# Niccolo-Ajroldi/plainLM

Hardware: AMD Instinct MI355X
Metric: tokens/sec fwd+bwd (160M, seq=1024, bf16) (higher is better)
Workload: dtype bf16

## Files before the change

plainlm_amd/_lib.py:

```python

import ctypes as C
import os
import re

_HERE = os.path.dirname(os.path.abspath(__file__))
LIB_PATH = os.path.join(_HERE, 'libplainlm_hip.so')
HEADER_PATH = os.path.join(os.path.dirname(_HERE), 'include', 'plainlm_hip.h')
EXT_HEADER_PATH = os.path.join(os.path.dirname(_HERE), 'include', 'plainlm_hip_ext.h')

_lib = None

EXPECTED_ABI = 112

_P = C.c_void_p
_I64 = C.c_int64
_I = C.c_int
_F = C.c_float
_SZ = C.c_size_t

class CastItem(C.Structure):
  _fields_ = [('src', _P), ('dst', _P), ('dst_t', _P), ('rows', _I64), ('cols', _I64), ('ld_t', _I64)]


class OptimItem(C.Structure):
  _fields_ = [('p', _P), ('g', _P), ('m', _P), ('v', _P), ('dst', _P), ('dst_t', _P), ('rows', _I64), ('cols', _I64), ('ld_t', _I64)]


class OptimHparams(C.Structure):
  _fields_ = [('kind', _I), ('first', _I), ('lr', _F), ('weight_decay', _F), ('decay', _F), ('beta1', _F), ('beta2', _F), ('eps', _F),
              ('momentum', _F), ('dampening', _F), ('bc2', _F), ('coef_grad', _F), ('coef_avg', _F),
              ('ckp1', _F), ('coef_y', _F), ('bc1', _F)]
# ... 72 lines not shown
  'plm_set_cu_reserve': (_I, [_I]),
  'plm_comm_unique_id': (_I, [_P]),
  'plm_comm_init': (_I, [C.POINTER(_P), _P, _I, _I, _I]),
  'plm_comm_init_capped': (_I, [C.POINTER(_P), _P, _I, _I, _I, _I]),
  'plm_comm_split': (_I, [_P, C.POINTER(_P), _I]),
  'plm_comm_destroy': (_I, [_P]),
  'plm_comm_allreduce_avg_f32': (_I, [_P, _P, _I64, _P]),
  'plm_comm_rsag_avg_f32': (_I, [_P, _P, _I64, _P]),
  'plm_comm_broadcast_f32': (_I, [_P, _P, _I64, _I, _P]),
  'plm_mx_quant': (_I, [_P, _I64, _I64, _I64, _P, _P, _P, _P, _P]),
  'plm_mx_quant_multi': (_I, [C.POINTER(MxQuantItem), _I, _P]),
  'plm_gemm_mx_nt': (_I, [_P, _P, _P, _P, _P, _I64, _I64, _I64, _I64, _I, _P]),
  'plm_probe_ds_read_tr16': (_I, [_P, _P]),
  'plm_probe_mfma32': (_I, [_P, _P, _P, _P]),
}


EXT_SIGNATURES = {
  'plm_head_predict_workspace_bytes': (_SZ, [_I64, _I64, _I64]),
  'plm_head_predict_bf16': (_I, [_P, _I64, _P, _I64, _P, _P, _P, _P, _P, _P, _I64, _I64, _I64, _P, _SZ, _P]),
}


def _declared(path):
  with open(path) as f:
    src = re.sub(r'/\*.*?\*/', '', f.read(), flags=re.S)
  return sorted(set(re.findall(r'\b(plm_[a-z0-9_]+)\s*\(', src)))


def header_functions():
  return _declared(HEADER_PATH)


def ext_header_functions():
  return _declared(EXT_HEADER_PATH)


def load():
  global _lib
  if _lib is not None:
    return _lib
  if not os.path.exists(LIB_PATH):
    raise RuntimeError(
      f'{LIB_PATH} not found: the HIP extension is not built. Run `make -C plainlm_amd/csrc` '
      '(or __graft_entry__.build()). plainlm_amd has no CPU fallback.')
  lib = C.CDLL(LIB_PATH, mode=C.RTLD_GLOBAL)
  for name, (res, args) in SIGNATURES.items():
    fn = getattr(lib, name)
    fn.restype = res
    fn.argtypes = args
  for name, (res, args) in EXT_SIGNATURES.items():
    fn = getattr(lib, name, None)
    if fn is None:
      raise RuntimeError(f'{LIB_PATH} lacks {name} (include/plainlm_hip_ext.h): rebuild it (make -C plainlm_amd/csrc)')
    fn.restype = res
    fn.argtypes = args
  got = lib.plm_version()
  if got != EXPECTED_ABI:
    raise RuntimeError(f'{LIB_PATH} reports ABI version {got}, this package was written for {EXPECTED_ABI}: '
                       'rebuild it (make -C plainlm_amd/csrc)')
  _lib = lib
  return lib


def check(rc, what):
  if rc != 0:
    msg = load().plm_last_error_string()
    raise RuntimeError(f'{what} failed (rc={rc}): {msg.decode() if msg else "?"}')
```

plainlm_amd/csrc/gemm_api.hip:

```cpp
#include <initializer_list>

#include "../../include/plainlm_hip_ext.h"
#include "gemm_launch.h"

static int g_num_cus = 0;
static int g_cu_reserve = 0;

extern "C" int plm_set_cu_reserve(int n) {
  if (n < 0 || n > 128) {
    plm_set_error("plm_set_cu_reserve: n=%d out of range 0..128", n);
    return PLM_E_INVALID;
  }
  g_cu_reserve = n;
  return PLM_OK;
}

static bool ensure_num_cus() {
  if (g_num_cus == 0) {
    int dev = 0;
    hipDeviceProp_t prop;
    if (hipGetDevice(&dev) != hipSuccess || hipGetDeviceProperties(&prop, dev) != hipSuccess) return false;
    g_num_cus = prop.multiProcessorCount > 0 ? prop.multiProcessorCount : 256;
  }
  return true;
}
// ... 103 lines not shown
    PLM_CHECK_LAUNCH("plm_fc1_swiglu_bf16");
    return PLM_OK;
  }
  if (int rc = plm_gemm_bf16_nt_ex(X, ldx, W, ldw, U, N, M, N, K, 0, 0, nullptr, 0, stream)) return rc;
  return plm_swiglu_fwd(U, ACT, M, h, stream);
}

extern "C" int plm_fc2_dx_swiglu_bwd_bf16(const uint16_t* dY, int64_t lddy, const uint16_t* W2T, int64_t ldw, const uint16_t* U, uint16_t* DU,
                                          uint16_t* scratch, int64_t M, int64_t h, int64_t K, void* stream) {
  PLM_REQUIRE(dY && W2T && U && DU, "plm_fc2_dx_swiglu_bwd_bf16: null pointer");
  PLM_REQUIRE(M > 0 && h > 0 && K > 0 && h % 8 == 0, "plm_fc2_dx_swiglu_bwd_bf16: bad shape (h %% 8 == 0)");
  if (lddy % 8 == 0 && ldw % 8 == 0 && aligned16({dY, W2T, DU}) && (reinterpret_cast<uintptr_t>(U) & 7) == 0 &&
      launch_nt_fused(NT_EPI_GLUB, GemmOperands{dY, lddy, W2T, ldw, DU, 2 * h, M, h, K, nullptr},
                      EpiArgs{const_cast<uint16_t*>(U), 2 * h, nullptr, nullptr, 0, 0}, stream)) {
    PLM_CHECK_LAUNCH("plm_fc2_dx_swiglu_bwd_bf16");
    return PLM_OK;
  }
  if (!scratch) {
    plm_set_error("plm_fc2_dx_swiglu_bwd_bf16: this shape (or PLM_GEMM_V1) takes the two-launch path and needs the M*h bf16 d(act) scratch");
    return PLM_E_WORKSPACE;
  }
  if (int rc = plm_gemm_bf16_nt_ex(dY, lddy, W2T, ldw, scratch, h, M, h, K, 0, 0, nullptr, 0, stream)) return rc;
  return plm_swiglu_bwd(scratch, U, DU, M, h, stream);
}

extern "C" size_t plm_gemm_tn_workspace_bytes(int64_t M, int64_t N, int64_t K) {
  const int slots = persistent_slots();
  if (M <= 0 || N <= 0 || K <= 0 || slots == 0) return 0;
  return tn_plan(M, N, K, slots, plan_env()).workspace_bytes;
}

extern "C" int plm_gemm_bf16_tn(const uint16_t* A, int64_t lda, const uint16_t* B, int64_t ldb, float* C, int64_t ldc, int64_t M,
                                int64_t N, int64_t K, int accumulate, const float* alpha_dev, void* workspace,
                                size_t workspace_bytes, void* stream) {
  PLM_REQUIRE(A && B && C, "plm_gemm_bf16_tn: null pointer");
  PLM_REQUIRE(M > 0 && N > 0 && K > 0 && M < (1 << 30) && N < (1 << 30) && K < (1 << 30), "plm_gemm_bf16_tn: bad shape M=%ld N=%ld K=%ld",
              (long)M, (long)N, (long)K);
  PLM_REQUIRE(M % 8 == 0 && N % 8 == 0 && lda % 8 == 0 && ldb % 8 == 0 && ldc % 4 == 0,
              "plm_gemm_bf16_tn: M, N, lda, ldb must be multiples of 8 and ldc of 4 (M=%ld N=%ld lda=%ld ldb=%ld ldc=%ld)", (long)M, (long)N,
              (long)lda, (long)ldb, (long)ldc);
  PLM_REQUIRE(((reinterpret_cast<uintptr_t>(A) | reinterpret_cast<uintptr_t>(B) | reinterpret_cast<uintptr_t>(C)) & 15) == 0,
              "plm_gemm_bf16_tn: base pointers must be 16-byte aligned");
  const int slots = persistent_slots();
  if (slots == 0) return PLM_E_HIP;
  const TnPlan p = tn_plan(M, N, K, slots, plan_env());
  if (p.splits > 1) {
// ... 166 lines not shown
```

plainlm_amd/csrc/gemm_big.hip:

```cpp
#include <stdlib.h>

#include <type_traits>
#include <utility>

#include "gemm_launch.h"

typedef __attribute__((address_space(3))) void lds_void_t;
typedef const __attribute__((address_space(1))) void gbl_void_t;

__device__ __forceinline__ void big_dma16(const void* gsrc, void* lds_wave_base) {
  __builtin_amdgcn_global_load_lds((gbl_void_t*)gsrc, (lds_void_t*)lds_wave_base, 16, 0, 0);
}
__device__ __forceinline__ int big_swz(int row, int chunk) { return row * 128 + ((chunk ^ ((row >> 1) & 7)) << 4); }

template <int N>
__device__ __forceinline__ void wait_vm() {
#ifdef PLM_DBG_DRAIN
  asm volatile("s_waitcnt vmcnt(0)" ::: "memory");
#else
  asm volatile("s_waitcnt vmcnt(%0)" ::"n"(N) : "memory");
#endif
}
template <int N0, int N1>
__device__ __forceinline__ void wait_vm_sel(int flag) {
// ... 75 lines not shown
    for (int u = 0; u < NUNIT; ++u)
      if (slot(u) == sl) return u;
    return -1;
  }
};
static_assert(NtOvlPlan<2, 3, 2>::slot(0) == 2 && NtOvlPlan<2, 3, 2>::slot(1) == 3 && NtOvlPlan<2, 3, 2>::slot(3) == 4 && NtOvlPlan<2, 3, 2>::slot(2) == 5,
              "256x192: (A0,B0) (A0,B1) (A1,B1) leave in phases 2 3 4, (A1,B0) behind the loop");
static_assert(NtOvlPlan<4, 2, 1>::slot(0) == 3 && NtOvlPlan<4, 2, 1>::slot(1) == 4 && NtOvlPlan<4, 2, 1>::slot(2) == 5 && NtOvlPlan<4, 2, 1>::slot(3) == 5,
              "256x256: the two pieces of A half 0 leave in phases 3 and 4");
static_assert(NtOvlPlan<1, 3, 2>::slot(1) == 4 && NtOvlPlan<1, 3, 2>::slot(0) == 5, "128x192: the B1 pass leaves in phase 4");

__device__ __forceinline__ float4 head_rec_combine(const float4 a, const float4 b) {
  const float m = fmaxf(a.x, b.x);
  const float ea_ = __expf(a.x - m), eb_ = __expf(b.x - m);
  const float sa = (a.x == -INFINITY) ? 0.f : a.y * ea_;
  const float sb = (b.x == -INFINITY) ? 0.f : b.y * eb_;
  const float ua = (a.x == -INFINITY) ? 0.f : ea_ * fmaf(a.y, a.x - m, a.z);
  const float ub = (b.x == -INFINITY) ? 0.f : eb_ * fmaf(b.y, b.x - m, b.z);
  const int ia = __float_as_int(a.w), ib = __float_as_int(b.w);
  const int idx = b.x > a.x ? ib : (b.x == a.x ? min(ia, ib) : ia);
  return make_float4(m, sa + sb, ua + ub, __int_as_float(idx));
}

template <int BM, int BN, int WM, int WN, bool HYB = false, bool GLU = false, bool GLUB = false, bool ROPE = false, bool SCORE = false>
__global__ __launch_bounds__(512, 2) void gemm_nt_big_kernel(const uint16_t* __restrict__ A, int64_t lda,
                                                             const uint16_t* __restrict__ B, int64_t ldb,
                                                             uint16_t* __restrict__ C, int64_t ldc, int M, int N, int K,
                                                             const float* __restrict__ alpha_dev, int tiles_m, int tiles_n,
                                                             HybridArgs hyb, EpiArgs ea) {
  uint16_t* const act = ea.act;
  const int64_t ldact = ea.ldact;
  static_assert(!(GLU || GLUB) || (BM == 256 && BN == 256 && WN == 4 && !HYB), "GLU epilogues: 256x256 tiles, whole-K items");
  static_assert(!(GLU && GLUB), "one epilogue at a time");
  static_assert(!SCORE || !(HYB || GLU || GLUB || ROPE), "SCORE: whole-K items, no other epilogue");
  constexpr int TM = BM / WM, TN = BN / WN;
  static_assert(WM * WN == 8 && (TN == 64 || TN == 96) && (TM == 128 || TM == 64 || TM == 32), "unsupported geometry");
  constexpr int AH = TM / 2;
  constexpr int NA = AH / 16;
  constexpr int BF0 = TN / 32 - 1, NBF = BF0 + 1;
  constexpr int A_ROWS = BM / 2, B0_ROWS = WN * 32 * BF0, B1_ROWS = WN * 32;
  constexpr int A_HT = A_ROWS * 128, B0_HT = B0_ROWS * 128, B1_HT = B1_ROWS * 128;
  constexpr int STAGE = 2 * A_HT + B0_HT + B1_HT;
  constexpr int A_DMA = A_ROWS / 64, B0_DMA = B0_ROWS / 64, B1_DMA = B1_ROWS / 64;
  static_assert(B0_DMA >= B1_DMA && B1_DMA >= 1, "half-tiles are whole DMA rounds of the workgroup");
  constexpr int OFF_A0 = 0, OFF_B0 = A_HT, OFF_B1 = A_HT + B0_HT, OFF_A1 = A_HT + B0_HT + B1_HT;
  constexpr int D_P4 = 2 * A_DMA + B0_DMA + 2 * B1_DMA;
  constexpr int D_P1 = 3 * A_DMA + B0_DMA + B1_DMA;
  constexpr int D_P2 = 3 * A_DMA + B0_DMA + B1_DMA;
  constexpr int NS = NA * 2 * NBF * (GLUB ? 2 : 1) + (GLU ? NA * 2 : 0);
  static_assert(D_P1 + NS < 64, "vmcnt is a 6-bit counter");
#ifndef PLM_NT_OVL
#define PLM_NT_OVL 1
#endif
  constexpr bool OVL = PLM_NT_OVL && !HYB && !GLU && !GLUB && !ROPE && !SCORE;
  using OP = NtOvlPlan<NA, NBF, BF0>;
  constexpr int NPASS = OP::NPASS, NUNIT = OP::NUNIT;
// ... 457 lines not shown
      auto drain = [&](auto utag) {
        constexpr int u = decltype(utag)::value;
        if (ovl && OP::slot(u) != 5) return;
        unit_write(utag);
        asm volatile("s_waitcnt lgkmcnt(0)" ::: "memory");
        unit_store(utag, std::false_type{}, m0, n0);
        asm volatile("s_waitcnt lgkmcnt(0)" ::: "memory");
      };
      nt_for_units(drain, std::make_integer_sequence<int, NUNIT>{});
      credit = m0 + BM <= M && n0 + BN <= N;
      credit_i = __builtin_amdgcn_readfirstlane(credit ? (ovl ? 2 : 1) : 0);
      continue;
    }
#pragma unroll
    for (int mf = 0; mf < NA; ++mf) {
      const int mrow0 = m0 + wm * TM + mf * 32;
      if (GLUB) {
        const uint16_t* u = act;
#pragma unroll
        for (int sr = 0; sr < 2; ++sr) {
          const int gm_l = min(mrow0 + sr * 16 + l15, M - 1);
          const int fi = 2 * mf + sr;
#pragma unroll
          for (int bq = 0; bq < 2; ++bq)
#pragma unroll
            for (int sc = 0; sc < 2; ++sc) {
              const int gn = n0 + wn * TN + bq * 32 + sc * 16 + 4 * q;
              const bf16x4_t xv = ld_bf16x4(u + (int64_t)gm_l * ldact + gn);
              const bf16x4_t zv = ld_bf16x4(u + (int64_t)gm_l * ldact + N + gn);
              bf16x4_t dxo, dzo;
#pragma unroll
              for (int e = 0; e < 4; ++e) {
                const float gf = bf2f(f2bf(acc4[fi][bq * 2 + sc][e]));
                const float xf = bf2f(xv[e]), zf = bf2f(zv[e]);
                const float sig = plm_sigmoid(xf);
                const bf16_t sv = f2bf(xf * sig);
                const bf16_t ds = f2bf(gf * zf);
                dzo[e] = f2bf(gf * bf2f(sv));
                dxo[e] = f2bf(bf2f(ds) * (sig * (1.f + xf * (1.f - sig))));
              }
              const int c = bq * 4 + sc * 2 + (q >> 1);
              *reinterpret_cast<bf16x4_t*>(epi + l15 * 128 + ((c ^ (l15 & 7)) << 4) + (q & 1) * 8) = dxo;
              *reinterpret_cast<bf16x4_t*>(epi + (16 + l15) * 128 + ((c ^ (l15 & 7)) << 4) + (q & 1) * 8) = dzo;
            }
          asm volatile("s_waitcnt lgkmcnt(0)" ::: "memory");
#pragma unroll
          for (int it = 0; it < 4; ++it) {
            const int c = it * 64 + lane;
            const int row = c >> 3, ch = c & 7;
            const bf16x8_t v = *reinterpret_cast<const bf16x8_t*>(epi + row * 128 + ((ch ^ (row & 7)) << 4));
            const int gm = mrow0 + sr * 16 + (row & 15);
            if (gm < M) st_c2_bf16x8(C + (int64_t)gm * ldc + (row >> 4) * N + n0 + wn * TN + ch * 8, v);
          }
          asm volatile("s_waitcnt lgkmcnt(0)" ::: "memory");
        }
        continue;
      }
#pragma unroll
      for (int p0 = 0; p0 < NBF; p0 += 2) {
        const int nb = NBF - p0 < 2 ? NBF - p0 : 2;
#pragma unroll
        for (int bq = 0; bq < 2; ++bq) {
          if (bq >= nb) continue;
          const int bh = p0 + bq;
#pragma unroll
          for (int sr = 0; sr < 2; ++sr)
#pragma unroll
            for (int sc = 0; sc < 2; ++sc) {
              bf16x4_t o;
#pragma unroll
              for (int e = 0; e < 4; ++e) o[e] = f2bf(acc4[2 * mf + sr][bh * 2 + sc][e]);
              const int row = sr * 16 + l15, c = bq * 4 + sc * 2 + (q >> 1);
              *reinterpret_cast<bf16x4_t*>(epi + row * 128 + ((c ^ (row & 7)) << 4) + (q & 1) * 8) = o;
            }
        }
        asm volatile("s_waitcnt lgkmcnt(0)" ::: "memory");
#pragma unroll
        for (int it = 0; it < 4; ++it) {
          if (it >= 2 * nb) continue;
          const int c = it * 64 + lane;
          const int row = nb == 2 ? c >> 3 : c >> 2, ch = nb == 2 ? c & 7 : c & 3;
          const bf16x8_t v = *reinterpret_cast<const bf16x8_t*>(epi + row * 128 + ((ch ^ (row & 7)) << 4));
// ... 424 lines not shown
  const int nq = N >> 3;
  const int64_t nv = (int64_t)rows * nq;
  const int64_t stride = (int64_t)gridDim.x * blockDim.x;
  for (int64_t i = (int64_t)blockIdx.x * blockDim.x + threadIdx.x; i < nv; i += stride) {
    const int64_t row = i / nq;
    const int col = (int)(i - row * nq) * 8;
    const int t = (int)(row >> 8) * tiles_n + (col >> 8);
    const int cf = (t * nkt) / L;
    const int cl = min(((t + 1) * nkt - 1) / L, nchunks - 1);
    f32x4_t a = *reinterpret_cast<const f32x4_t*>(ws + row * N + col);
    f32x4_t b = *reinterpret_cast<const f32x4_t*>(ws + row * N + col + 4);
    for (int k = 1; k <= cl - cf; ++k) {
      a += *reinterpret_cast<const f32x4_t*>(ws + ((int64_t)k * rows + row) * N + col);
      b += *reinterpret_cast<const f32x4_t*>(ws + ((int64_t)k * rows + row) * N + col + 4);
    }
    u32x4_t o = {pack_bf2(a[0] * alpha, a[1] * alpha), pack_bf2(a[2] * alpha, a[3] * alpha), pack_bf2(b[0] * alpha, b[1] * alpha),
                 pack_bf2(b[2] * alpha, b[3] * alpha)};
    *reinterpret_cast<u32x4_t*>(C + row * ldc + col) = o;
  }
}

template <NtEpilogue EPI, bool HYB, int BM, int BN, int WM, int WN>
static void nt_launch_tile(const NtPlan& p, const GemmOperands& o, float* slabs, const EpiArgs& ea, hipStream_t s) {
  hipLaunchKernelGGL((gemm_nt_big_kernel<BM, BN, WM, WN, HYB, EPI == NT_EPI_GLU, EPI == NT_EPI_GLUB, EPI == NT_EPI_ROPE, EPI == NT_EPI_SCORE>),
                     dim3((unsigned)p.grid), dim3(512), 0, s, o.A, o.lda, o.B, o.ldb, (uint16_t*)o.C, o.ldc, (int)o.M, (int)o.N, (int)o.K, o.alpha_dev, p.tm,
                     p.tn, HybridArgs{p.rfull, p.nchunks, p.L, slabs}, ea);
}

template <NtEpilogue EPI>
static void nt_launch(const NtPlan& p, const GemmOperands& o, float* slabs, const EpiArgs& ea, hipStream_t s) {
  if constexpr (EPI == NT_EPI_NONE) {
    if (p.kernel == NT_HYBRID) {
      nt_launch_tile<EPI, true, 256, 256, 2, 4>(p, o, slabs, ea, s);
      const int64_t rem_rows = o.M - (int64_t)p.rfull * 256;
      const int64_t nv = rem_rows * (o.N / 8);
      int64_t rb = plm_cdiv(nv, 256);
      if (rb > 4096) rb = 4096;
      hipLaunchKernelGGL(nt_streamk_reduce_kernel, dim3((unsigned)rb), dim3(256), 0, s, (const float*)slabs,
                         (uint16_t*)o.C + (int64_t)p.rfull * 256 * o.ldc, o.ldc, (int)rem_rows, (int)o.N, p.tn, (int)(o.K / 64), p.L, p.nchunks, o.alpha_dev);
      return;
    }
  }
  if (p.tile == 0) nt_launch_tile<EPI, false, 256, 256, 2, 4>(p, o, nullptr, ea, s);
  if constexpr (EPI != NT_EPI_GLU && EPI != NT_EPI_GLUB) {
    if (p.tile == 1) nt_launch_tile<EPI, false, 256, 128, 4, 2>(p, o, nullptr, ea, s);
    else if (p.tile == 2) nt_launch_tile<EPI, false, 256, 192, 4, 2>(p, o, nullptr, ea, s);
    else if (p.tile == 3) nt_launch_tile<EPI, false, 128, 192, 4, 2>(p, o, nullptr, ea, s);
  }
}

void plm_launch_gemm_nt_persistent(const NtPlan& p, NtEpilogue epilogue, const GemmOperands& o, float* slabs, const EpiArgs& ea, hipStream_t s) {
  switch (epilogue) {
    case NT_EPI_NONE: return nt_launch<NT_EPI_NONE>(p, o, slabs, ea, s);
    case NT_EPI_ROPE: return nt_launch<NT_EPI_ROPE>(p, o, slabs, ea, s);
    case NT_EPI_GLU: return nt_launch<NT_EPI_GLU>(p, o, slabs, ea, s);
    case NT_EPI_GLUB: return nt_launch<NT_EPI_GLUB>(p, o, slabs, ea, s);
    case NT_EPI_SCORE: return nt_launch<NT_EPI_SCORE>(p, o, slabs, ea, s);
  }
}

__global__ __launch_bounds__(256) void head_score_combine_kernel(const float* __restrict__ part, const float* __restrict__ xt,
                                                                 const int64_t* __restrict__ targets, float* __restrict__ nll,
                                                                 float* __restrict__ lse_out, int M, int V, int ntc) {
  __shared__ float2 sh[8][32];
  const int r = threadIdx.x & 31, sl = threadIdx.x >> 5;
  const int row = blockIdx.x * 32 + r;
  float m = -INFINITY, s = 0.f;
  if (row < M) {
    for (int tc = sl; tc < ntc; tc += 8) {
      const float2 b = *reinterpret_cast<const float2*>(part + 2 * ((int64_t)tc * M + row));
      const float mm = fmaxf(m, b.x);
      const float sa = (m == -INFINITY) ? 0.f : s * __expf(m - mm);
      const float sb = (b.x == -INFINITY) ? 0.f : b.y * __expf(b.x - mm);
      m = mm;
      s = sa + sb;
    }
  }
  sh[sl][r] = make_float2(m, s);
  __syncthreads();
  if (sl != 0 || row >= M) return;
#pragma unroll
// ... 117 lines not shown
```

plainlm_amd/csrc/gemm_launch.h:

```cpp
#pragma once

#include "gemm_plan.h"
#include "plm_device.h"

struct EpiArgs {
  uint16_t* act;
  int64_t ldact;
  const float* rcos;
  const float* rsin;
  int T, rope_cols;
  const int64_t* targets;
  float* part;
  float* xt;
  float* part4;
};

struct GemmOperands {
  const uint16_t* A;
  int64_t lda;
  const uint16_t* B;
  int64_t ldb;
  void* C;
  int64_t ldc, M, N, K;
  const float* alpha_dev;
};

void plm_launch_gemm_nt_128(const NtPlan& p, const GemmOperands& o, int c_dtype, int accumulate, hipStream_t s);
void plm_launch_gemm_tn_128(const TnPlan& p, const GemmOperands& o, int accumulate, float* slabs, hipStream_t s);
void plm_launch_splitk_reduce(const TnPlan& p, const GemmOperands& o, int accumulate, float* slabs, hipStream_t s);

void plm_launch_gemm_nt_persistent(const NtPlan& p, NtEpilogue epilogue, const GemmOperands& o, float* slabs, const EpiArgs& ea, hipStream_t s);
void plm_launch_gemm_tn_persistent(const TnPlan& p, const GemmOperands& o, int accumulate, float* slabs, hipStream_t s);
void plm_launch_gemm_tn_grouped(const TnGroup& g, const TnGroupOut& out, int64_t K, float* ws, int slots, hipStream_t s);
void plm_launch_head_score_combine(const float* part, const float* xt, const int64_t* targets, float* nll, float* lse, int64_t M, int64_t V, int ntc,
                                   hipStream_t s);
void plm_launch_head_score_rows(const uint16_t* logits, int64_t ld, const int64_t* targets, float* nll, float* lse, int64_t rows, int64_t V,
                                hipStream_t s);
struct HeadPredictOut {
  int64_t* pred;
  float *logp, *entropy, *nll, *lse;
};
void plm_launch_head_predict_combine(const float* part4, const float* xt, const int64_t* targets, const HeadPredictOut& out, int64_t M, int64_t V,
                                     int ntc, hipStream_t s);
void plm_launch_head_predict_rows(const uint16_t* logits, int64_t ld, const int64_t* targets, const HeadPredictOut& out, int64_t rows, int64_t V,
                                  hipStream_t s);
```

plainlm_amd/csrc/gemm_plan.h:

```cpp
#pragma once

#include <stddef.h>
#include <stdint.h>

static inline int64_t plan_cdiv(int64_t a, int64_t b) { return (a + b - 1) / b; }

struct GemmPlanEnv {
  bool gemm_v1, tn_no_big, nt_no_hybrid;
  long long nt_hybrid_min_k;
};

static inline double round_efficiency(int64_t tiles, int slots) {
  const int64_t rounds = (tiles + slots - 1) / slots;
  return (double)tiles / (double)(rounds * slots);
}

struct NtTileShape {
  int bm, bn;
  double rate;
};
static const NtTileShape kNtTiles[4] = {{256, 256, 1.0}, {256, 128, 0.88}, {256, 192, 0.94}, {128, 192, 0.72}};
static const int kNtTileVariant[4] = {4, 6, 5, 7};
static inline double nt_tile_eff(int i, int64_t M, int64_t N, int slots) {
  const NtTileShape& t = kNtTiles[i];
  const int64_t tm = plan_cdiv(M, t.bm), tn = plan_cdiv(N, t.bn);
  return round_efficiency(tm * tn, slots) * ((double)N / (double)(tn * t.bn)) * ((double)M / (double)(tm * t.bm)) * t.rate;
}
static inline int nt_pick_tile(int64_t M, int64_t N, int slots, double* eff) {
  int best = 0;
  double be = -1.0;
  for (int i = 0; i < 4; ++i) {
    const double e = nt_tile_eff(i, M, N, slots);
    if (e > be) {
      be = e;
      best = i;
    }
  }
  *eff = be;
  return best;
}
static inline double nt_dma128_eff(int64_t M, int64_t N, int slots) {
  const int64_t tm = plan_cdiv(M, 128), tn = plan_cdiv(N, 128);
  return round_efficiency(tm * tn, 2 * slots) * ((double)N / (double)(tn * 128)) * ((double)M / (double)(tm * 128)) * 0.80;
}

static inline bool nt_dma_shape(int64_t N, int64_t K, int64_t ldc) { return (K % 64 == 0) && (N % 8 == 0) && (ldc % 8 == 0); }

enum NtEpilogue { NT_EPI_NONE, NT_EPI_ROPE, NT_EPI_GLU, NT_EPI_GLUB, NT_EPI_SCORE };
enum NtKernel {
  NT_REG128,
  NT_DMA128,
  NT_PERSISTENT,
  NT_HYBRID
};
struct NtPlan {
  bool ok;
  NtKernel kernel;
  int tile;
  int tm, tn, grid;
  int rfull, nchunks, L;
  size_t workspace_bytes;
};

static inline bool nt_hybrid_plan(int64_t M, int64_t N, int64_t K, int slots, const GemmPlanEnv& env, NtPlan* p) {
  if (env.nt_no_hybrid) return false;
  const bool mk = env.nt_hybrid_min_k >= 0;
  const int64_t min_k = mk ? env.nt_hybrid_min_k : 8192, min_l = mk ? 2 : 8;
  if (K % 64 != 0 || N % 8 != 0 || M < 2048 || N < 256 || K < min_k) return false;
  const int64_t R = plan_cdiv(M, 256), Cn = plan_cdiv(N, 256), tiles = R * Cn, nkt = K / 64;
  if (tiles <= slots) return false;
  if (round_efficiency(tiles, slots) >= 0.9) return false;
// ... 8 lines not shown
  if (L < min_l || L * 10 > nkt * 9) return false;
  p->rfull = (int)rf;
  p->L = (int)L;
  p->nchunks = (int)plan_cdiv(total, L);
  const int64_t nslabs = (nkt - 1) / L + 2;
  p->workspace_bytes = (size_t)nslabs * (size_t)(M - rf * 256) * (size_t)N * sizeof(float);
  return true;
}

static inline NtPlan nt_plan(int64_t M, int64_t N, int64_t K, int64_t ldc, int c_dtype, int variant, bool have_workspace, NtEpilogue epilogue,
                             int slots, const GemmPlanEnv& env) {
  NtPlan p{};
  p.ok = true;
  auto persistent = [&](int tile) {
    p.kernel = NT_PERSISTENT;
    p.tile = tile;
    p.tm = (int)plan_cdiv(M, kNtTiles[tile].bm);
    p.tn = (int)plan_cdiv(N, kNtTiles[tile].bn);
    p.grid = p.tm * p.tn < slots ? p.tm * p.tn : slots;
    p.rfull = p.tm;
    p.nchunks = 0;
    p.L = 1;
  };
  if (epilogue == NT_EPI_GLU || epilogue == NT_EPI_GLUB) {
    p.ok = !env.gemm_v1 && K % 64 == 0 && N % 256 == 0 && M >= 512;
    if (p.ok) persistent(0);
    return p;
  }
  const bool dma_ok = variant >= 2 || (variant == 0 && !env.gemm_v1 && nt_dma_shape(N, K, ldc));
  if (variant >= 3) {
    for (int i = 0; i < 4; ++i)
      if (kNtTileVariant[i] == (variant == 3 ? 4 : variant)) persistent(i);
    return p;
  }
  if (variant == 0 && dma_ok && c_dtype == 0) {
    if (have_workspace && epilogue == NT_EPI_NONE && nt_hybrid_plan(M, N, K, slots, env, &p)) {
      p.kernel = NT_HYBRID;
      p.tm = (int)plan_cdiv(M, 256);
      p.tn = (int)plan_cdiv(N, 256);
      const int nitems = p.rfull * p.tn + p.nchunks;
      p.grid = nitems < slots ? nitems : slots;
      return p;
    }
    double eff;
    const int tile = nt_pick_tile(M, N, slots, &eff);
    if (M >= 512 && N >= 128 && eff >= nt_dma128_eff(M, N, slots)) {
      persistent(tile);
      return p;
// ... 127 lines not shown
```

plainlm_amd/functional.py:

```python

import torch

from . import ops


class GradSink:

  def __init__(self):
    self.enabled = False
    self.written = set()
    self.on_ready = None
    self.on_queued = None
    self.dw_group_local, self.dw_group_ddp = 48, 12
    self.dw_queue_bytes_max = None
    self.dw_queue_bytes = 0
    self.dw_queue = []
    self.norm_queue = []

  def begin_window(self):
    self.flush_dw()
    self.written.clear()

  def defer_dw(self, dy, x, p):
    mx = isinstance(dy, ops.MxTensor) and isinstance(x, ops.MxTensor)
# ... 75 lines not shown
  def forward(ctx, x, weight, lin):
    wb, _ = lin.shadow()
    ctx.save_for_backward(x)
    ctx.lin = lin
    return ops.gemm_nt(x, wb)

  @staticmethod
  def backward(ctx, dy):
    (x,) = ctx.saved_tensors
    lin = ctx.lin
    dy = dy.contiguous()
    _, wbt = lin.shadow()
    dx = ops.gemm_nt(dy, wbt[:, :lin.out_features]) if ctx.needs_input_grad[0] else None
    dw = None
    if ctx.needs_input_grad[1]:
      sink, p = lin.sink, lin.weight
      if sink is not None and sink.active_for(p):
        sink.defer_dw(dy, x, p)
      else:
        dw = ops.gemm_tn(dy, x)
    return dx, dw, None


class SwiGLUMLPFn(torch.autograd.Function):

  @staticmethod
  def forward(ctx, x, w1, w2, fc1, fc2):
    w1b, _ = fc1.shadow()
    w2b, _ = fc2.shadow()
    u, act = ops.fc1_swiglu(x, w1b)
    ctx.save_for_backward(x, u, act)
    ctx.fc1, ctx.fc2 = fc1, fc2
    return ops.gemm_nt(act, w2b)

  @staticmethod
  def backward(ctx, dy):
    x, u, act = ctx.saved_tensors
    fc1, fc2 = ctx.fc1, ctx.fc2
    dy = dy.contiguous()
    _, w1t = fc1.shadow()
    _, w2t = fc2.shadow()
    du = ops.fc2_dx_swiglu_bwd(dy, w2t[:, :fc2.out_features], u)
    dw2 = dw1 = None
    if ctx.needs_input_grad[2]:
      sink, p = fc2.sink, fc2.weight
      if sink is not None and sink.active_for(p):
        sink.defer_dw(dy, act, p)
      else:
        dw2 = ops.gemm_tn(dy, act)
    dx = ops.gemm_nt(du, w1t[:, :fc1.out_features]) if ctx.needs_input_grad[0] else None
    if ctx.needs_input_grad[1]:
      sink, p = fc1.sink, fc1.weight
      if sink is not None and sink.active_for(p):
        sink.defer_dw(du, x, p)
      else:
        dw1 = ops.gemm_tn(du, x)
    return dx, dw1, dw2, None, None


class PlainMLPFn(torch.autograd.Function):

  @staticmethod
  def forward(ctx, x, w1, w2, fc1, fc2, kind):
    w1b, _ = fc1.shadow()
    w2b, _ = fc2.shadow()
# ... 354 lines not shown
```

plainlm_amd/ops.py:

```python

import collections
import ctypes as C
import os

import torch

from . import _lib

BF16 = torch.bfloat16
F32 = torch.float32


def _stream():
  return C.c_void_p(torch.cuda.current_stream().cuda_stream)


PROFILE = None
LAUNCH_HOOK = None


class _Timed:
  __slots__ = ('family', 'flops', 'start')

  def __init__(self, family, flops):
# ... 429 lines not shown
  return u, act


def fc2_dx_swiglu_bwd(dy, w2t, u):
  _need(dy, BF16, 'fc2_dx_swiglu_bwd.dy', 2)
  _need(w2t, BF16, 'fc2_dx_swiglu_bwd.w2t', 2)
  _need(u, BF16, 'fc2_dx_swiglu_bwd.u', 2)
  M, K = dy.shape
  h = w2t.shape[0]
  if w2t.shape[1] != K or u.shape != (M, 2 * h) or not u.is_contiguous() or dy.stride(1) != 1 or w2t.stride(1) != 1:
    raise ValueError('fc2_dx_swiglu_bwd: need dy [M, K], w2t [h, K], contiguous u [M, 2h]')
  du = torch.empty((M, 2 * h), dtype=BF16, device=dy.device)
  lib = _lib.load()
  _hook('gemm_nt_fused', 2.0 * M * h * K)
  with _Timed('gemm_nt_fused', 2.0 * M * h * K):
    rc = lib.plm_fc2_dx_swiglu_bwd_bf16(_p(dy), dy.stride(0), _p(w2t), w2t.stride(0), _p(u), _p(du), _p(None), M, h, K, _stream())
    if rc == -4:
      scratch = torch.empty((M, h), dtype=BF16, device=dy.device)
      rc = lib.plm_fc2_dx_swiglu_bwd_bf16(_p(dy), dy.stride(0), _p(w2t), w2t.stride(0), _p(u), _p(du), _p(scratch), M, h, K, _stream())
    _lib.check(rc, 'plm_fc2_dx_swiglu_bwd_bf16')
  return du


def rope_qk_(qkv, rope_cos, rope_sin, B, T, nh):
  _need(qkv, BF16, 'rope_qk.qkv', 2)
  hd = qkv.shape[1] // (3 * nh)
  _need(rope_cos, F32, 'rope_qk.rope_cos', 2)
  _need(rope_sin, F32, 'rope_qk.rope_sin', 2)
  if rope_cos.shape[0] < T or rope_cos.shape[1] != hd // 2:
    raise ValueError('rope_qk: RoPE table too short for T or wrong head_dim')
  _lib.check(_lib.load().plm_rope_qk(_p(qkv), _p(rope_cos), _p(rope_sin), B, T, nh, hd, _stream()), 'plm_rope_qk')
  return qkv


def qkv_rope(x, w_qkv, rope_cos, rope_sin, B, T, nh):
  _need(x, BF16, 'qkv_rope.x', 2)
  _need(w_qkv, BF16, 'qkv_rope.w', 2)
  M, K = x.shape
  N = w_qkv.shape[0]
  hd = N // (3 * nh)
  out = torch.empty((M, N), dtype=BF16, device=x.device)
  _hook('gemm_nt_fused', 2.0 * M * N * K)
  with _Timed('gemm_nt_fused', 2.0 * M * N * K):
    _lib.check(_lib.load().plm_qkv_rope_bf16(_p(x), x.stride(0), _p(w_qkv), w_qkv.stride(0), _p(out), N, M, K, _p(rope_cos),
                                             _p(rope_sin), B, T, nh, hd, _stream()), 'plm_qkv_rope_bf16')
  return out
# ... 316 lines not shown
```

Before: 1.065 million.

## Save fc1 SwiGLU output in a tile-packed layout matching the backward epilogue

Adds packed-layout variants of the fused fc1+SwiGLU forward GEMM and the fc2 dx+SwiGLU backward GEMM. The forward epilogue writes the pre-activation u per wave and lane in 1 KiB units, so the backward epilogue can read gate and up values with contiguous 16-byte loads instead of strided row loads. This is meant to cut uncoalesced global reads and store work in the GLU epilogues. It is on by default when the shape qualifies, pads M up to a multiple of 256 in the saved buffer, and adds an unpack kernel for consumers that need the plain layout.

```diff
diff --git a/include/plainlm_hip_packed.h b/include/plainlm_hip_packed.h
--- /dev/null
+++ b/include/plainlm_hip_packed.h
@@ -0,0 +1,22 @@
+#ifndef PLAINLM_HIP_PACKED_H
+#define PLAINLM_HIP_PACKED_H
+
+#include "plainlm_hip.h"
+
+#ifdef __cplusplus
+extern "C" {
+#endif
+
+size_t plm_swiglu_packed_bytes(int64_t M, int64_t h);
+int plm_swiglu_packed_ok(int64_t M, int64_t h, int64_t K_fc1, int64_t K_fc2);
+int plm_fc1_swiglu_packed_bf16(const uint16_t* X, int64_t ldx, const uint16_t* W, int64_t ldw, uint16_t* PACKED, uint16_t* ACT, int64_t M,
+                               int64_t h, int64_t K, int max_workgroups, void* stream);
+int plm_fc2_dx_swiglu_bwd_packed_bf16(const uint16_t* dY, int64_t lddy, const uint16_t* W2T, int64_t ldw, const uint16_t* PACKED,
+                                      uint16_t* DU, int64_t M, int64_t h, int64_t K, int max_workgroups, void* stream);
+int plm_swiglu_unpack_bf16(const uint16_t* PACKED, uint16_t* U, int64_t M, int64_t h, void* stream);
+
+#ifdef __cplusplus
+}
+#endif
+
+#endif
diff --git a/plainlm_amd/_lib.py b/plainlm_amd/_lib.py
--- a/plainlm_amd/_lib.py
+++ b/plainlm_amd/_lib.py
@@ -7,6 +7,7 @@
 LIB_PATH = os.path.join(_HERE, 'libplainlm_hip.so')
 HEADER_PATH = os.path.join(os.path.dirname(_HERE), 'include', 'plainlm_hip.h')
 EXT_HEADER_PATH = os.path.join(os.path.dirname(_HERE), 'include', 'plainlm_hip_ext.h')
+PACKED_HEADER_PATH = os.path.join(os.path.dirname(_HERE), 'include', 'plainlm_hip_packed.h')
 
 _lib = None
 
@@ -125,6 +126,15 @@
 }
 
 
+PACKED_SIGNATURES = {
+  'plm_swiglu_packed_bytes': (_SZ, [_I64, _I64]),
+  'plm_swiglu_packed_ok': (_I, [_I64, _I64, _I64, _I64]),
+  'plm_fc1_swiglu_packed_bf16': (_I, [_P, _I64, _P, _I64, _P, _P, _I64, _I64, _I64, _I, _P]),
+  'plm_fc2_dx_swiglu_bwd_packed_bf16': (_I, [_P, _I64, _P, _I64, _P, _P, _I64, _I64, _I64, _I, _P]),
+  'plm_swiglu_unpack_bf16': (_I, [_P, _P, _I64, _I64, _P]),
+}
+
+
 def _declared(path):
   with open(path) as f:
     src = re.sub(r'/\*.*?\*/', '', f.read(), flags=re.S)
@@ -137,6 +147,10 @@
 
 def ext_header_functions():
   return _declared(EXT_HEADER_PATH)
+
+
+def packed_header_functions():
+  return _declared(PACKED_HEADER_PATH)
 
 
 def load():
@@ -152,12 +166,13 @@
     fn = getattr(lib, name)
     fn.restype = res
     fn.argtypes = args
-  for name, (res, args) in EXT_SIGNATURES.items():
-    fn = getattr(lib, name, None)
-    if fn is None:
-      raise RuntimeError(f'{LIB_PATH} lacks {name} (include/plainlm_hip_ext.h): rebuild it (make -C plainlm_amd/csrc)')
-    fn.restype = res
-    fn.argtypes = args
+  for header, table in (('plainlm_hip_ext.h', EXT_SIGNATURES), ('plainlm_hip_packed.h', PACKED_SIGNATURES)):
+    for name, (res, args) in table.items():
+      fn = getattr(lib, name, None)
+      if fn is None:
+        raise RuntimeError(f'{LIB_PATH} lacks {name} (include/{header}): rebuild it (make -C plainlm_amd/csrc)')
+      fn.restype = res
+      fn.argtypes = args
   got = lib.plm_version()
   if got != EXPECTED_ABI:
     raise RuntimeError(f'{LIB_PATH} reports ABI version {got}, this package was written for {EXPECTED_ABI}: '
diff --git a/plainlm_amd/csrc/gemm_api.hip b/plainlm_amd/csrc/gemm_api.hip
--- a/plainlm_amd/csrc/gemm_api.hip
+++ b/plainlm_amd/csrc/gemm_api.hip
@@ -1,6 +1,7 @@
 #include <initializer_list>
 
 #include "../../include/plainlm_hip_ext.h"
+#include "../../include/plainlm_hip_packed.h"
 #include "gemm_launch.h"
 
 static int g_num_cus = 0;
@@ -150,6 +151,66 @@
   }
   if (int rc = plm_gemm_bf16_nt_ex(dY, lddy, W2T, ldw, scratch, h, M, h, K, 0, 0, nullptr, 0, stream)) return rc;
   return plm_swiglu_bwd(scratch, U, DU, M, h, stream);
+}
+
+static bool launch_nt_packed(NtEpilogue epilogue, const GemmOperands& o, const EpiArgs& ea, int max_workgroups, void* stream) {
+  const int slots = persistent_slots();
+  if (slots == 0) return false;
+  NtPlan p = nt_plan(o.M, o.N, o.K, o.ldc, 0, 0, false, epilogue, slots, plan_env());
+  if (!p.ok) {
+    plm_set_error("packed SwiGLU GEMM: needs K %% 64 == 0, h %% 256 == 0 and the LDS-DMA kernels (no PLM_GEMM_V1); M=%ld N=%ld K=%ld", (long)o.M, (long)o.N,
+                  (long)o.K);
+    return false;
+  }
+  if (max_workgroups > 0 && max_workgroups < p.grid) p.grid = max_workgroups;
+  plm_launch_gemm_nt_persistent(p, epilogue, o, nullptr, ea, (hipStream_t)stream);
+  return true;
+}
+
+extern "C" size_t plm_swiglu_packed_bytes(int64_t M, int64_t h) { return (M > 0 && h > 0 && h % 128 == 0) ? glu_packed_bytes(M, h) : 0; }
+
+extern "C" int plm_swiglu_packed_ok(int64_t M, int64_t h, int64_t K_fc1, int64_t K_fc2) {
+  const int slots = persistent_slots();
+  if (slots == 0 || M <= 0 || h <= 0 || K_fc1 <= 0 || K_fc2 <= 0) return 0;
+  return nt_plan(M, 2 * h, K_fc1, 2 * h, 0, 0, false, NT_EPI_GLU, slots, plan_env()).ok &&
+         nt_plan(M, h, K_fc2, 2 * h, 0, 0, false, NT_EPI_GLUB, slots, plan_env()).ok;
+}
+
+extern "C" int plm_fc1_swiglu_packed_bf16(const uint16_t* X, int64_t ldx, const uint16_t* W, int64_t ldw, uint16_t* PACKED, uint16_t* ACT, int64_t M,
+                                          int64_t h, int64_t K, int max_workgroups, void* stream) {
+  PLM_REQUIRE(X && W && PACKED && ACT, "plm_fc1_swiglu_packed_bf16: null pointer");
+  PLM_REQUIRE(M > 0 && h > 0 && K > 0 && M < (1 << 30) && h < (1 << 29) && K < (1 << 30) && h % 128 == 0,
+              "plm_fc1_swiglu_packed_bf16: bad shape (h %% 128 == 0)");
+  PLM_REQUIRE(ldx % 8 == 0 && ldw % 8 == 0 && ldx >= K && ldw >= K && aligned16({X, W, PACKED, ACT}),
+              "plm_fc1_swiglu_packed_bf16: row strides must be multiples of 8 and >= K, pointers 16-byte aligned");
+  if (!launch_nt_packed(NT_EPI_GLU_PACKED, GemmOperands{X, ldx, W, ldw, PACKED, 2 * h, M, 2 * h, K, nullptr}, EpiArgs{ACT, h, nullptr, nullptr, 0, 0},
+                        max_workgroups, stream))
+    return PLM_E_INVALID;
+  PLM_CHECK_LAUNCH("plm_fc1_swiglu_packed_bf16");
+  return PLM_OK;
+}
+
+extern "C" int plm_fc2_dx_swiglu_bwd_packed_bf16(const uint16_t* dY, int64_t lddy, const uint16_t* W2T, int64_t ldw, const uint16_t* PACKED,
+                                                 uint16_t* DU, int64_t M, int64_t h, int64_t K, int max_workgroups, void* stream) {
+  PLM_REQUIRE(dY && W2T && PACKED && DU, "plm_fc2_dx_swiglu_bwd_packed_bf16: null pointer");
+  PLM_REQUIRE(M > 0 && h > 0 && K > 0 && M < (1 << 30) && h < (1 << 29) && K < (1 << 30) && h % 256 == 0,
+              "plm_fc2_dx_swiglu_bwd_packed_bf16: bad shape (h %% 256 == 0)");
+  PLM_REQUIRE(lddy % 8 == 0 && ldw % 8 == 0 && lddy >= K && ldw >= K && aligned16({dY, W2T, PACKED, DU}),
+              "plm_fc2_dx_swiglu_bwd_packed_bf16: row strides must be multiples of 8 and >= K, pointers 16-byte aligned");
+  if (!launch_nt_packed(NT_EPI_GLUB_PACKED, GemmOperands{dY, lddy, W2T, ldw, DU, 2 * h, M, h, K, nullptr},
+                        EpiArgs{const_cast<uint16_t*>(PACKED), 2 * h, nullptr, nullptr, 0, 0}, max_workgroups, stream))
+    return PLM_E_INVALID;
+  PLM_CHECK_LAUNCH("plm_fc2_dx_swiglu_bwd_packed_bf16");
+  return PLM_OK;
+}
+
+extern "C" int plm_swiglu_unpack_bf16(const uint16_t* PACKED, uint16_t* U, int64_t M, int64_t h, void* stream) {
+  PLM_REQUIRE(PACKED && U, "plm_swiglu_unpack_bf16: null pointer");
+  PLM_REQUIRE(M > 0 && h > 0 && M < (1 << 30) && h < (1 << 29) && h % 128 == 0, "plm_swiglu_unpack_bf16: bad shape (h %% 128 == 0)");
+  PLM_REQUIRE(aligned16({PACKED}) && (reinterpret_cast<uintptr_t>(U) & 7) == 0, "plm_swiglu_unpack_bf16: PACKED must be 16-byte aligned, U 8-byte");
+  plm_launch_swiglu_unpack(PACKED, U, M, h, (hipStream_t)stream);
+  PLM_CHECK_LAUNCH("plm_swiglu_unpack_bf16");
+  return PLM_OK;
 }
 
 extern "C" size_t plm_gemm_tn_workspace_bytes(int64_t M, int64_t N, int64_t K) {
diff --git a/plainlm_amd/csrc/gemm_big.hip b/plainlm_amd/csrc/gemm_big.hip
--- a/plainlm_amd/csrc/gemm_big.hip
+++ b/plainlm_amd/csrc/gemm_big.hip
@@ -121,7 +121,7 @@
   return make_float4(m, sa + sb, ua + ub, __int_as_float(idx));
 }
 
-template <int BM, int BN, int WM, int WN, bool HYB = false, bool GLU = false, bool GLUB = false, bool ROPE = false, bool SCORE = false>
+template <int BM, int BN, int WM, int WN, bool PK = false, bool HYB = false, bool GLU = false, bool GLUB = false, bool ROPE = false, bool SCORE = false>
 __global__ __launch_bounds__(512, 2) void gemm_nt_big_kernel(const uint16_t* __restrict__ A, int64_t lda,
                                                              const uint16_t* __restrict__ B, int64_t ldb,
                                                              uint16_t* __restrict__ C, int64_t ldc, int M, int N, int K,
@@ -131,6 +131,7 @@
   const int64_t ldact = ea.ldact;
   static_assert(!(GLU || GLUB) || (BM == 256 && BN == 256 && WN == 4 && !HYB), "GLU epilogues: 256x256 tiles, whole-K items");
   static_assert(!(GLU && GLUB), "one epilogue at a time");
+  static_assert(!PK || GLU || GLUB, "PK: the packed layout of the saved fc1 output");
   static_assert(!SCORE || !(HYB || GLU || GLUB || ROPE), "SCORE: whole-K items, no other epilogue");
   constexpr int TM = BM / WM, TN = BN / WN;
   static_assert(WM * WN == 8 && (TN == 64 || TN == 96) && (TM == 128 || TM == 64 || TM == 32), "unsupported geometry");
@@ -634,17 +635,29 @@
           const int gm_l = min(mrow0 + sr * 16 + l15, M - 1);
           const int fi = 2 * mf + sr;
 #pragma unroll
-          for (int bq = 0; bq < 2; ++bq)
+          for (int bq = 0; bq < 2; ++bq) {
+            u32x4_t pg = {0u, 0u, 0u, 0u}, pu = {0u, 0u, 0u, 0u};
+            if constexpr (PK) {
+              const char* blk = reinterpret_cast<const char*>(u) +
+                                glu_packed_unit_offset(m0 / BM, 2 * (n0 / BN) + (wn >> 1), 2 * tiles_n, wm * WN + (wn & 1) * 2 + bq, mf * 4 + sr * 2);
+              pg = *reinterpret_cast<const u32x4_t*>(blk + lane * 16);
+              pu = *reinterpret_cast<const u32x4_t*>(blk + kGluPackedUnitBytes + lane * 16);
+            }
 #pragma unroll
             for (int sc = 0; sc < 2; ++sc) {
               const int gn = n0 + wn * TN + bq * 32 + sc * 16 + 4 * q;
-              const bf16x4_t xv = ld_bf16x4(u + (int64_t)gm_l * ldact + gn);
-              const bf16x4_t zv = ld_bf16x4(u + (int64_t)gm_l * ldact + N + gn);
+              bf16x4_t xv, zv;
+              if constexpr (!PK) {
+                xv = ld_bf16x4(u + (int64_t)gm_l * ldact + gn);
+                zv = ld_bf16x4(u + (int64_t)gm_l * ldact + N + gn);
+              }
               bf16x4_t dxo, dzo;
 #pragma unroll
               for (int e = 0; e < 4; ++e) {
                 const float gf = bf2f(f2bf(acc4[fi][bq * 2 + sc][e]));
-                const float xf = bf2f(xv[e]), zf = bf2f(zv[e]);
+                const unsigned wg = pg[sc * 2 + (e >> 1)], wu = pu[sc * 2 + (e >> 1)];
+                const float xf = PK ? ((e & 1) ? bf_hi(wg) : bf_lo(wg)) : bf2f(xv[e]);
+                const float zf = PK ? ((e & 1) ? bf_hi(wu) : bf_lo(wu)) : bf2f(zv[e]);
                 const float sig = plm_sigmoid(xf);
                 const bf16_t sv = f2bf(xf * sig);
                 const bf16_t ds = f2bf(gf * zf);
@@ -655,6 +668,7 @@
               *reinterpret_cast<bf16x4_t*>(epi + l15 * 128 + ((c ^ (l15 & 7)) << 4) + (q & 1) * 8) = dxo;
               *reinterpret_cast<bf16x4_t*>(epi + (16 + l15) * 128 + ((c ^ (l15 & 7)) << 4) + (q & 1) * 8) = dzo;
             }
+          }
           asm volatile("s_waitcnt lgkmcnt(0)" ::: "memory");
 #pragma unroll
           for (int it = 0; it < 4; ++it) {
@@ -668,8 +682,22 @@
         }
         continue;
       }
-#pragma unroll
-      for (int p0 = 0; p0 < NBF; p0 += 2) {
+      if constexpr (GLU && PK) {
+        char* blk = reinterpret_cast<char*>(C) + glu_packed_unit_offset(m0 / BM, n0 / BN, tiles_n, wave, mf * 4) + lane * 16;
+#pragma unroll
+        for (int sr = 0; sr < 2; ++sr)
+#pragma unroll
+          for (int g = 0; g < 2; ++g) {
+            bf16x8_t o;
+#pragma unroll
+            for (int sc = 0; sc < 2; ++sc)
+#pragma unroll
+              for (int e = 0; e < 4; ++e) o[sc * 4 + e] = f2bf(acc4[2 * mf + sr][2 * g + sc][e]);
+            st_c_bf16x8(reinterpret_cast<uint16_t*>(blk + (sr * 2 + g) * kGluPackedUnitBytes), o);
+          }
+      }
+#pragma unroll
+      for (int p0 = 0; p0 < (GLU && PK ? 0 : NBF); p0 += 2) {
         const int nb = NBF - p0 < 2 ? NBF - p0 : 2;
 #pragma unroll
         for (int bq = 0; bq < 2; ++bq) {
@@ -1140,7 +1168,9 @@
 
 template <NtEpilogue EPI, bool HYB, int BM, int BN, int WM, int WN>
 static void nt_launch_tile(const NtPlan& p, const GemmOperands& o, float* slabs, const EpiArgs& ea, hipStream_t s) {
-  hipLaunchKernelGGL((gemm_nt_big_kernel<BM, BN, WM, WN, HYB, EPI == NT_EPI_GLU, EPI == NT_EPI_GLUB, EPI == NT_EPI_ROPE, EPI == NT_EPI_SCORE>),
+  constexpr bool PK = EPI == NT_EPI_GLU_PACKED || EPI == NT_EPI_GLUB_PACKED;
+  hipLaunchKernelGGL((gemm_nt_big_kernel<BM, BN, WM, WN, PK, HYB, EPI == NT_EPI_GLU || EPI == NT_EPI_GLU_PACKED, EPI == NT_EPI_GLUB || EPI == NT_EPI_GLUB_PACKED,
+                                         EPI == NT_EPI_ROPE, EPI == NT_EPI_SCORE>),
                      dim3((unsigned)p.grid), dim3(512), 0, s, o.A, o.lda, o.B, o.ldb, (uint16_t*)o.C, o.ldc, (int)o.M, (int)o.N, (int)o.K, o.alpha_dev, p.tm,
                      p.tn, HybridArgs{p.rfull, p.nchunks, p.L, slabs}, ea);
 }
@@ -1160,7 +1190,7 @@
     }
   }
   if (p.tile == 0) nt_launch_tile<EPI, false, 256, 256, 2, 4>(p, o, nullptr, ea, s);
-  if constexpr (EPI != NT_EPI_GLU && EPI != NT_EPI_GLUB) {
+  if constexpr (EPI != NT_EPI_GLU && EPI != NT_EPI_GLUB && EPI != NT_EPI_GLU_PACKED && EPI != NT_EPI_GLUB_PACKED) {
     if (p.tile == 1) nt_launch_tile<EPI, false, 256, 128, 4, 2>(p, o, nullptr, ea, s);
     else if (p.tile == 2) nt_launch_tile<EPI, false, 256, 192, 4, 2>(p, o, nullptr, ea, s);
     else if (p.tile == 3) nt_launch_tile<EPI, false, 128, 192, 4, 2>(p, o, nullptr, ea, s);
@@ -1174,7 +1204,30 @@
     case NT_EPI_GLU: return nt_launch<NT_EPI_GLU>(p, o, slabs, ea, s);
     case NT_EPI_GLUB: return nt_launch<NT_EPI_GLUB>(p, o, slabs, ea, s);
     case NT_EPI_SCORE: return nt_launch<NT_EPI_SCORE>(p, o, slabs, ea, s);
-  }
+    case NT_EPI_GLU_PACKED: return nt_launch<NT_EPI_GLU_PACKED>(p, o, slabs, ea, s);
+    case NT_EPI_GLUB_PACKED: return nt_launch<NT_EPI_GLUB_PACKED>(p, o, slabs, ea, s);
+  }
+}
+
+__global__ __launch_bounds__(256) void swiglu_unpack_kernel(const uint16_t* __restrict__ packed, uint16_t* __restrict__ U, int M, int h, int tiles_n,
+                                                            int64_t nchunks) {
+  const int64_t i = (int64_t)blockIdx.x * blockDim.x + threadIdx.x;
+  if (i >= nchunks) return;
+  const int lane = (int)(i & 63), unit = (int)(i >> 6) & 15, wave = (int)(i >> 10) & 7;
+  const int64_t tile = i >> 13;
+  const int tm = (int)(tile / tiles_n), tn = (int)(tile % tiles_n);
+  const int row = tm * 256 + (wave >> 2) * 128 + (unit >> 2) * 32 + ((unit >> 1) & 1) * 16 + (lane & 15);
+  if (row >= M) return;
+  const u32x4_t v = *reinterpret_cast<const u32x4_t*>(reinterpret_cast<const char*>(packed) + i * 16);
+  uint16_t* dst = U + (int64_t)row * (2 * h) + (unit & 1) * h + tn * 128 + (wave & 3) * 32 + 4 * (lane >> 4);
+  *reinterpret_cast<u32x2_t*>(dst) = u32x2_t{v[0], v[1]};
+  *reinterpret_cast<u32x2_t*>(dst + 16) = u32x2_t{v[2], v[3]};
+}
+
+void plm_launch_swiglu_unpack(const uint16_t* packed, uint16_t* U, int64_t M, int64_t h, hipStream_t s) {
+  const int tiles_n = (int)(2 * h / 256);
+  const int64_t nchunks = plm_cdiv(M, 256) * tiles_n * (int64_t)(kGluPackedWaves * kGluPackedUnits * 64);
+  hipLaunchKernelGGL(swiglu_unpack_kernel, dim3((unsigned)plm_cdiv(nchunks, 256)), dim3(256), 0, s, packed, U, (int)M, (int)h, tiles_n, nchunks);
 }
 
 __global__ __launch_bounds__(256) void head_score_combine_kernel(const float* __restrict__ part, const float* __restrict__ xt,
diff --git a/plainlm_amd/csrc/gemm_launch.h b/plainlm_amd/csrc/gemm_launch.h
--- a/plainlm_amd/csrc/gemm_launch.h
+++ b/plainlm_amd/csrc/gemm_launch.h
@@ -2,6 +2,12 @@
 
 #include "gemm_plan.h"
 #include "plm_device.h"
+
+static constexpr int kGluPackedUnitBytes = 1024, kGluPackedUnits = 16, kGluPackedWaves = 8;
+__host__ __device__ inline int64_t glu_packed_unit_offset(int tile_m, int tile_n, int tiles_n, int wave, int unit) {
+  return ((((int64_t)tile_m * tiles_n + tile_n) * kGluPackedWaves + wave) * kGluPackedUnits + unit) * kGluPackedUnitBytes;
+}
+static inline size_t glu_packed_bytes(int64_t M, int64_t h) { return (size_t)(plm_cdiv(M, 256) * 256) * (size_t)(2 * h) * sizeof(uint16_t); }
 
 struct EpiArgs {
   uint16_t* act;
@@ -30,6 +36,7 @@
 void plm_launch_splitk_reduce(const TnPlan& p, const GemmOperands& o, int accumulate, float* slabs, hipStream_t s);
 
 void plm_launch_gemm_nt_persistent(const NtPlan& p, NtEpilogue epilogue, const GemmOperands& o, float* slabs, const EpiArgs& ea, hipStream_t s);
+void plm_launch_swiglu_unpack(const uint16_t* packed, uint16_t* U, int64_t M, int64_t h, hipStream_t s);
 void plm_launch_gemm_tn_persistent(const TnPlan& p, const GemmOperands& o, int accumulate, float* slabs, hipStream_t s);
 void plm_launch_gemm_tn_grouped(const TnGroup& g, const TnGroupOut& out, int64_t K, float* ws, int slots, hipStream_t s);
 void plm_launch_head_score_combine(const float* part, const float* xt, const int64_t* targets, float* nll, float* lse, int64_t M, int64_t V, int ntc,
diff --git a/plainlm_amd/csrc/gemm_plan.h b/plainlm_amd/csrc/gemm_plan.h
--- a/plainlm_amd/csrc/gemm_plan.h
+++ b/plainlm_amd/csrc/gemm_plan.h
@@ -46,7 +46,7 @@
 
 static inline bool nt_dma_shape(int64_t N, int64_t K, int64_t ldc) { return (K % 64 == 0) && (N % 8 == 0) && (ldc % 8 == 0); }
 
-enum NtEpilogue { NT_EPI_NONE, NT_EPI_ROPE, NT_EPI_GLU, NT_EPI_GLUB, NT_EPI_SCORE };
+enum NtEpilogue { NT_EPI_NONE, NT_EPI_ROPE, NT_EPI_GLU, NT_EPI_GLUB, NT_EPI_SCORE, NT_EPI_GLU_PACKED, NT_EPI_GLUB_PACKED };
 enum NtKernel {
   NT_REG128,
   NT_DMA128,
@@ -101,8 +101,9 @@
     p.nchunks = 0;
     p.L = 1;
   };
-  if (epilogue == NT_EPI_GLU || epilogue == NT_EPI_GLUB) {
-    p.ok = !env.gemm_v1 && K % 64 == 0 && N % 256 == 0 && M >= 512;
+  const bool packed = epilogue == NT_EPI_GLU_PACKED || epilogue == NT_EPI_GLUB_PACKED;
+  if (epilogue == NT_EPI_GLU || epilogue == NT_EPI_GLUB || packed) {
+    p.ok = !env.gemm_v1 && K % 64 == 0 && N % 256 == 0 && (packed || M >= 512);
     if (p.ok) persistent(0);
     return p;
   }
diff --git a/plainlm_amd/functional.py b/plainlm_amd/functional.py
--- a/plainlm_amd/functional.py
+++ b/plainlm_amd/functional.py
@@ -121,13 +121,17 @@
     return dx, dw, None
 
 
+PACKED_SWIGLU = True
+
+
 class SwiGLUMLPFn(torch.autograd.Function):
 
   @staticmethod
   def forward(ctx, x, w1, w2, fc1, fc2):
     w1b, _ = fc1.shadow()
     w2b, _ = fc2.shadow()
-    u, act = ops.fc1_swiglu(x, w1b)
+    ctx.packed = PACKED_SWIGLU and ops.swiglu_packed_ok(x.shape[0], w1b.shape[0] // 2, x.shape[1], fc2.out_features)
+    u, act = ops.fc1_swiglu_packed(x, w1b) if ctx.packed else ops.fc1_swiglu(x, w1b)
     ctx.save_for_backward(x, u, act)
     ctx.fc1, ctx.fc2 = fc1, fc2
     return ops.gemm_nt(act, w2b)
@@ -139,7 +143,7 @@
     dy = dy.contiguous()
     _, w1t = fc1.shadow()
     _, w2t = fc2.shadow()
-    du = ops.fc2_dx_swiglu_bwd(dy, w2t[:, :fc2.out_features], u)
+    du = (ops.fc2_dx_swiglu_bwd_packed if ctx.packed else ops.fc2_dx_swiglu_bwd)(dy, w2t[:, :fc2.out_features], u)
     dw2 = dw1 = None
     if ctx.needs_input_grad[2]:
       sink, p = fc2.sink, fc2.weight
diff --git a/plainlm_amd/ops.py b/plainlm_amd/ops.py
--- a/plainlm_amd/ops.py
+++ b/plainlm_amd/ops.py
@@ -475,6 +475,54 @@
   return du
 
 
+def swiglu_packed_ok(M, h, k_fc1, k_fc2):
+  return bool(_lib.load().plm_swiglu_packed_ok(int(M), int(h), int(k_fc1), int(k_fc2)))
+
+
+def fc1_swiglu_packed(x, w_fc1, max_workgroups=0):
+  _need(x, BF16, 'fc1_swiglu_packed.x', 2)
+  _need(w_fc1, BF16, 'fc1_swiglu_packed.w', 2)
+  M, K = x.shape
+  N = w_fc1.shape[0]
+  if w_fc1.shape[1] != K or N % 256 != 0 or x.stride(1) != 1 or w_fc1.stride(1) != 1:
+    raise ValueError('fc1_swiglu_packed: need x [M, K], w [2h, K] with unit inner strides and h % 128 == 0')
+  h = N // 2
+  packed = torch.empty(((M + 255) // 256 * 256, N), dtype=BF16, device=x.device)
+  act = torch.empty((M, h), dtype=BF16, device=x.device)
+  _hook('gemm_nt_fused', 2.0 * M * N * K)
+  with _Timed('gemm_nt_fused', 2.0 * M * N * K):
+    _lib.check(_lib.load().plm_fc1_swiglu_packed_bf16(_p(x), x.stride(0), _p(w_fc1), w_fc1.stride(0), _p(packed), _p(act), M, h, K,
+                                                      int(max_workgroups), _stream()), 'plm_fc1_swiglu_packed_bf16')
+  return packed, act
+
+
+def fc2_dx_swiglu_bwd_packed(dy, w2t, packed, max_workgroups=0):
+  _need(dy, BF16, 'fc2_dx_swiglu_bwd_packed.dy', 2)
+  _need(w2t, BF16, 'fc2_dx_swiglu_bwd_packed.w2t', 2)
+  _need(packed, BF16, 'fc2_dx_swiglu_bwd_packed.packed', 2)
+  M, K = dy.shape
+  h = w2t.shape[0]
+  if (w2t.shape[1] != K or h % 256 != 0 or packed.shape != ((M + 255) // 256 * 256, 2 * h) or not packed.is_contiguous() or dy.stride(1) != 1
+      or w2t.stride(1) != 1):
+    raise ValueError('fc2_dx_swiglu_bwd_packed: need dy [M, K], w2t [h, K] with h % 256 == 0, packed from fc1_swiglu_packed')
+  du = torch.empty((M, 2 * h), dtype=BF16, device=dy.device)
+  _hook('gemm_nt_fused', 2.0 * M * h * K)
+  with _Timed('gemm_nt_fused', 2.0 * M * h * K):
+    _lib.check(_lib.load().plm_fc2_dx_swiglu_bwd_packed_bf16(_p(dy), dy.stride(0), _p(w2t), w2t.stride(0), _p(packed), _p(du), M, h, K,
+                                                             int(max_workgroups), _stream()), 'plm_fc2_dx_swiglu_bwd_packed_bf16')
+  return du
+
+
+def swiglu_unpack(packed, M):
+  _need(packed, BF16, 'swiglu_unpack.packed', 2)
+  N = packed.shape[1]
+  if N % 256 != 0 or packed.shape[0] != (M + 255) // 256 * 256 or not packed.is_contiguous():
+    raise ValueError('swiglu_unpack: need the packed buffer of fc1_swiglu_packed and its M')
+  u = torch.empty((M, N), dtype=BF16, device=packed.device)
+  _lib.check(_lib.load().plm_swiglu_unpack_bf16(_p(packed), _p(u), M, N // 2, _stream()), 'plm_swiglu_unpack_bf16')
+  return u
+
+
 def rope_qk_(qkv, rope_cos, rope_sin, B, T, nh):
   _need(qkv, BF16, 'rope_qk.qkv', 2)
   hd = qkv.shape[1] // (3 * nh)
```

After: 1.073 million, median of 6. Within noise of the previous version (+0.8%).
